# qwerty35/swarm_simulator

Hardware: AMD Instinct MI355X
Metric: agent-trajectories/sec (RBP plan: SFC+RSFC+QP) (higher is better)
Workload: dtype f64

## Files before the change

swarm_simulator_amd/csrc/kernels/knot_lds.inc:

```
#pragma once
#include "knot_panel_layout.h"

#define KL_LD 38
#define KL_LDU 50
#define KL_I 40
#ifndef KL_XCH
#define KL_XCH 6
#endif
typedef __attribute__((address_space(3))) double kl_lds;
typedef __attribute__((address_space(3))) int kl_ldsi;
typedef double kl_d2 __attribute__((ext_vector_type(2)));
typedef __attribute__((address_space(3))) kl_d2 kl_lds2;
typedef double kl_d4 __attribute__((ext_vector_type(4)));

__host__ __device__ constexpr int kl_area_doubles(int nk) {
    return ((nk + 1) * KL_LDU + (nk + 1) * KL_LD + KL_I + 1) & ~1;
}

template <int NK>
struct KlArea {
    static constexpr int NT = (NK + 15) / 16;
    static constexpr int C = 0, CSZ = (NK + 1) * KL_LDU;
    static constexpr int MX = CSZ, MXSZ = (NK + 1) * KL_LD;
    static constexpr int I = MX + MXSZ;
// ... 122 lines not shown
    }
}

#ifndef KL_FOLLOW_STRIDE
#define KL_FOLLOW_STRIDE 2
#endif
template <int NK>
__device__ __forceinline__ void kl_follow_LinvT(double (&m)[NK], const kl_lds* C, const kl_lds* I, kl_ldsi* P, int pbase) {
    double v[NK];
    kl_await_opaque(P, pbase + (KL_FOLLOW_STRIDE + 1 < NK ? KL_FOLLOW_STRIDE + 1 : NK));
    kl_load_tail<NK>(v, C, 1);
#pragma unroll
    for (int c = 0; c + 1 < NK; ++c) {
        if (c > 0 && c % KL_FOLLOW_STRIDE == 0) kl_await_opaque(P, pbase + (c + KL_FOLLOW_STRIDE + 1 < NK ? c + KL_FOLLOW_STRIDE + 1 : NK));
        const double s = m[c] * I[c];
        kl_axpy_roll<NK>(m, s, v, c + 1, C + (c + 1) * KL_LD, c + 2, c + 2 < NK);
    }
}

template <int NK>
__device__ __forceinline__ void kl_store_rows(const double (&m)[NK], kl_lds* MX, int r, bool act) {
    kl_lds* row = MX + (act ? r : NK) * KL_LD;
#pragma unroll
    for (int k = 0; k + 1 < NK; k += 2) *(kl_lds2*)(row + k) = kl_d2{m[k], m[k + 1]};
    if (NK & 1) row[NK - 1] = m[NK - 1];
    kl_sync();
}

template <int NK>
__device__ __forceinline__ void kl_coupling_rows(double (&x)[NK], kl_lds* MX, int r, bool act, double e0, double e1, double e2) {
    const int g3 = 3 * ((act ? r : 0) / 3);
    const kl_lds* m0 = MX + g3 * KL_LD;
    constexpr int NP = NK / 2;
    kl_d2 t[2][3][KL_XCH];
#pragma unroll
    for (int p = 0; p < KL_XCH && p < NP; ++p)
#pragma unroll
        for (int q = 0; q < 3; ++q) t[0][q][p] = *(const kl_lds2*)(m0 + q * KL_LD + 2 * p);
#pragma unroll
    for (int ch = 0; ch * KL_XCH < NP; ++ch) {
#pragma unroll
        for (int p = 0; p < KL_XCH; ++p)
            if ((ch + 1) * KL_XCH + p < NP)
#pragma unroll
                for (int q = 0; q < 3; ++q) t[(ch + 1) & 1][q][p] = *(const kl_lds2*)(m0 + q * KL_LD + 2 * ((ch + 1) * KL_XCH + p));
#pragma unroll
        for (int p = 0; p < KL_XCH; ++p) {
            const int k = 2 * (ch * KL_XCH + p);
            if (k + 1 < NK) {
                x[k] = e0 * t[ch & 1][0][p][0] + e1 * t[ch & 1][1][p][0] + e2 * t[ch & 1][2][p][0];
                x[k + 1] = e0 * t[ch & 1][0][p][1] + e1 * t[ch & 1][1][p][1] + e2 * t[ch & 1][2][p][1];
            }
        }
    }
    if (NK & 1) x[NK - 1] = e0 * m0[NK - 1] + e1 * m0[KL_LD + NK - 1] + e2 * m0[2 * KL_LD + NK - 1];
    kl_sync();
    kl_store_rows<NK>(x, MX, r, act);
}

template <int NK>
__device__ __forceinline__ void kl_syrk(const kl_lds* MX, const kl_lds* I, kl_lds* U, int lane, bool accumulate) {
    constexpr int NT = (NK + 15) / 16, KS = (NK + 3) / 4;
    const int li = lane & 15, lk = lane >> 4;
#pragma unroll
    for (int ti = 0; ti < NT; ++ti) {
        kl_d4 acc[NT];
#pragma unroll
        for (int t = 0; t < NT; ++t) acc[t] = kl_d4{0, 0, 0, 0};
        for (int ks = (3 * ((16 * ti) / 3)) / 4; ks < KS; ++ks) {
            const int kc = 4 * ks + lk;
            const double dk = kc < NK ? I[kc] : 0.0;
            const double opi = (kc < NK ? MX[(16 * ti + li < NK ? 16 * ti + li : NK) * KL_LD + kc] : 0.0) * dk;
#pragma unroll
            for (int tj = 0; tj <= ti; ++tj) {
                const double opj = kc < NK ? MX[(16 * tj + li < NK ? 16 * tj + li : NK) * KL_LD + kc] : 0.0;
                acc[tj] = __builtin_amdgcn_mfma_f64_16x16x4f64(opi, opj, acc[tj], 0, 0, 0);
            }
        }
#pragma unroll
        for (int tj = 0; tj <= ti; ++tj)
#pragma unroll
            for (int g = 0; g < 4; ++g) {
                const int row = 16 * ti + lk + 4 * g;
                kl_lds* u = U + (row < NK ? row : NK) * KL_LDU + 16 * tj + li;
                *u = accumulate ? *u + acc[tj][g] : acc[tj][g];
            }
    }
    kl_sync();
}

#ifndef KL_PANEL
#define KL_PANEL 1
#endif
#ifndef KL_PANEL_MIN_NK
#define KL_PANEL_MIN_NK 36
#endif
__host__ __device__ constexpr bool kl_panel_path(int nk) { return KL_PANEL && nk >= KL_PANEL_MIN_NK; }

template <int NK>
struct KlPanels {
    static constexpr int NT = kp_nt(NK), NP = kp_np(NK), TILES = kp_ntiles(NT);
    static_assert(kp_img_total(NK) <= KlArea<NK>::CSZ, "the panel images must fit the C / U region");
};

__device__ __forceinline__ double kl_recip(double d) {
    const double inv = __builtin_amdgcn_rcp(d);
    return __builtin_fma(__builtin_fma(-d, inv, 1.0), inv, inv);
}
__device__ __forceinline__ double kl_pick(bool c, double a, double b) {
    const long long m = -(long long)c;
    return __longlong_as_double((__double_as_longlong(a) & m) | (__double_as_longlong(b) & ~m));
}
__device__ __forceinline__ double kl_sel4(const double (&v)[4], int k) {
    return kl_pick((k & 2) != 0, kl_pick((k & 1) != 0, v[3], v[2]), kl_pick((k & 1) != 0, v[1], v[0]));
}

struct KlPivot {
    double d0, d10, d11, d20, d21, d22, d30, d31, d32, d33;
    double i0, i1, i2, i3;
    double w10, w20, w21, w30, w31, w32;
    double l10, l20, l21, l30, l31, l32;
    bool ok;
};
__device__ __forceinline__ void kl_pivot_load(KlPivot& f, const kl_lds* img, int p) {
    const kl_lds* b = img + kp_img_entry(KP_W * p, 0);
    f.d0 = b[0];
    const kl_d2 r1 = *(const kl_lds2*)(b + 4), r2 = *(const kl_lds2*)(b + 8), r3 = *(const kl_lds2*)(b + 12), r3b = *(const kl_lds2*)(b + 14);
    f.d22 = b[10];
    f.d10 = r1[0], f.d11 = r1[1], f.d20 = r2[0], f.d21 = r2[1], f.d30 = r3[0], f.d31 = r3[1], f.d32 = r3b[0], f.d33 = r3b[1];
}
__device__ __forceinline__ void kl_pivot_factor(KlPivot& f) {
    f.i0 = kl_recip(f.d0);
    f.w10 = f.d10, f.l10 = f.w10 * f.i0;
    f.w20 = f.d20, f.l20 = f.w20 * f.i0;
    f.w30 = f.d30, f.l30 = f.w30 * f.i0;
    const double d1 = __builtin_fma(-f.l10, f.w10, f.d11);
    f.i1 = kl_recip(d1);
    f.w21 = __builtin_fma(-f.l20, f.w10, f.d21), f.l21 = f.w21 * f.i1;
    f.w31 = __builtin_fma(-f.l30, f.w10, f.d31), f.l31 = f.w31 * f.i1;
    const double d2 = __builtin_fma(-f.l21, f.w21, __builtin_fma(-f.l20, f.w20, f.d22));
    f.i2 = kl_recip(d2);
    f.w32 = __builtin_fma(-f.l31, f.w21, __builtin_fma(-f.l30, f.w20, f.d32)), f.l32 = f.w32 * f.i2;
    const double d3 = __builtin_fma(-f.l32, f.w32, __builtin_fma(-f.l31, f.w31, __builtin_fma(-f.l30, f.w30, f.d33)));
    f.i3 = kl_recip(d3);
    f.ok = f.d0 > 0 && d1 > 0 && d2 > 0 && d3 > 0;
}
__device__ __forceinline__ void kl_panel_row(const KlPivot& f, const kl_d2 s01, const kl_d2 s23, double (&L)[4], double (&W)[4]) {
    W[0] = s01[0], L[0] = W[0] * f.i0;
    W[1] = __builtin_fma(-L[0], f.w10, s01[1]), L[1] = W[1] * f.i1;
    W[2] = __builtin_fma(-L[1], f.w21, __builtin_fma(-L[0], f.w20, s23[0])), L[2] = W[2] * f.i2;
    W[3] = __builtin_fma(-L[2], f.w32, __builtin_fma(-L[1], f.w31, __builtin_fma(-L[0], f.w30, s23[1]))), L[3] = W[3] * f.i3;
}

template <int NK, bool SUB, bool BOTH, class F>
__device__ __forceinline__ void kl_tiles_load(kl_d4 (&s)[KlPanels<NK>::TILES], int lane, F&& entry) {
    constexpr int NT = KlPanels<NK>::NT;
    const int li = lane & 15, lk = lane >> 4;
#pragma unroll
    for (int ti = 0; ti < NT; ++ti)
#pragma unroll
        for (int tj = ti; tj < NT; ++tj)
#pragma unroll
            for (int g = 0; g < 4; ++g) {
                const int i = KP_T * ti + lk + 4 * g, j = KP_T * tj + li;
                const int mx = BOTH ? j : i > j ? i : j, mn = BOTH ? i : i > j ? j : i;
                const bool full = KP_T * tj + KP_T <= NK;
                const bool pad = !full && (i >= NK || j >= NK);
                const double v = entry(full || mx < NK ? mx : NK - 1, full || mn < NK ? mn : NK - 1);
                const int tile = kp_upper(ti, tj, NT);
                if (SUB)
                    s[tile][g] -= pad ? 0.0 : v;
                else
                    s[tile][g] = pad ? (i == j ? 1.0 : 0.0) : v;
            }
}

template <int NK>
__device__ __forceinline__ void kl_panel_out(const kl_d4 (&s)[KlPanels<NK>::TILES], kl_lds* C, int p, int li, int lk) {
    constexpr int NT = KlPanels<NK>::NT;
    kl_lds* img = C + kp_img_off(NK, p);
#pragma unroll
    for (int tj = 0; tj < NT; ++tj)
        if (tj >= kp_panel_tile(p)) img[kp_img_entry(KP_T * tj + li, lk)] = s[kp_upper(kp_panel_tile(p), tj, NT)][kp_panel_reg(p)];
}

template <int NK>
__device__ __forceinline__ void kl_rows_load(kl_d2 (&raw)[KlPanels<NK>::NT][2], const kl_lds* img, int t_first, int li) {
#pragma unroll
    for (int t = 0; t < KlPanels<NK>::NT; ++t)
        if (t >= t_first) raw[t][0] = *(const kl_lds2*)(img + kp_img_entry(KP_T * t + li, 0)), raw[t][1] = *(const kl_lds2*)(img + kp_img_entry(KP_T * t + li, 2));
}

template <int NK>
__device__ __forceinline__ bool kl_ldl_panels(kl_d4 (&s)[KlPanels<NK>::TILES], kl_lds* C, kl_lds* I, int lane, kl_ldsi* P, int pbase) {
    constexpr int NT = KlPanels<NK>::NT, NP = KlPanels<NK>::NP;
    const int li = lane & 15, lk = lane >> 4;
    bool ok = true;
    KlPivot f;
    kl_d2 raw[NT][2];
    kl_panel_out<NK>(s, C, 0, li, lk);
    kl_sync();
    kl_pivot_load(f, C, 0);
    kl_rows_load<NK>(raw, C, 0, li);
#pragma unroll
    for (int p = 0; p < NP; ++p) {
        const int tc = kp_panel_tile(p), t0 = kp_first_live_tile(p);
        kl_lds* img = C + kp_img_off(NK, p);
        kl_pivot_factor(f);
        ok = ok && f.ok;
        if (KP_W * p + 0 < NK) I[KP_W * p + 0] = f.i0;
        if (KP_W * p + 1 < NK) I[KP_W * p + 1] = f.i1;
        if (KP_W * p + 2 < NK) I[KP_W * p + 2] = f.i2;
        if (KP_W * p + 3 < NK) I[KP_W * p + 3] = f.i3;
        const double inv[4] = {f.i0, f.i1, f.i2, f.i3};
        const double isel = kl_sel4(inv, lk);
        double a[NT], b[NT];
#pragma unroll
        for (int t = 0; t < NT; ++t)
            if (t >= tc) {
                double L[4], W[4];
                kl_panel_row(f, raw[t][0], raw[t][1], L, W);
                b[t] = kl_sel4(W, lk);
                const double l = b[t] * isel;
                a[t] = -l;
                img[kp_img_entry(KP_T * t + li, lk)] = l;
            }
        if (p + 1 < NP) {
#pragma unroll
            for (int tj = 0; tj < NT; ++tj)
                if (tj >= t0) s[kp_upper(t0, tj, NT)] = __builtin_amdgcn_mfma_f64_16x16x4f64(a[t0], b[tj], s[kp_upper(t0, tj, NT)], 0, 0, 0);
        }
        kl_sync();
        kl_publish(P, pbase + p + 1);
        if (p + 1 < NP) {
            kl_panel_out<NK>(s, C, p + 1, li, lk);
            kl_sync();
            kl_pivot_load(f, C + kp_img_off(NK, p + 1), p + 1);
            kl_rows_load<NK>(raw, C + kp_img_off(NK, p + 1), kp_panel_tile(p + 1), li);
            __builtin_amdgcn_sched_barrier(0);
#pragma unroll
            for (int ti = 0; ti < NT; ++ti)
#pragma unroll
                for (int tj = ti; tj < NT; ++tj)
                    if (ti > t0) s[kp_upper(ti, tj, NT)] = __builtin_amdgcn_mfma_f64_16x16x4f64(a[ti], b[tj], s[kp_upper(ti, tj, NT)], 0, 0, 0);
        }
    }
    kl_publish(P, pbase + NK + 1);
    return ok;
}

template <int NK, bool T_BOTH, class TF, class LF>
__device__ __forceinline__ bool kl_knot_panels(TF&& t_entry, LF&& t_loaded, bool minus_u, kl_lds* C, kl_lds* I, int lane, kl_ldsi* P, int pbase) {
    kl_d4 s[KlPanels<NK>::TILES];
    kl_tiles_load<NK, false, T_BOTH>(s, lane, t_entry);
    t_loaded();
    if (minus_u) kl_tiles_load<NK, true, true>(s, lane, [&](int mx, int mn) { return (double)C[mx * KL_LDU + mn]; });
    kl_sync();
    return kl_ldl_panels<NK>(s, C, I, lane, P, pbase);
}

template <int NK, bool WAIT>
__device__ __forceinline__ void kl_inverse_panels(kl_d4 (&n)[KlPanels<NK>::TILES], const kl_lds* C, int lane, kl_ldsi* P, int pbase) {
    constexpr int NT = KlPanels<NK>::NT, NP = KlPanels<NK>::NP;
    const int li = lane & 15, lk = lane >> 4;
#pragma unroll
    for (int ti = 0; ti < NT; ++ti)
#pragma unroll
        for (int tj = 0; tj <= ti; ++tj)
#pragma unroll
            for (int g = 0; g < 4; ++g) n[kp_lower(ti, tj)][g] = (ti == tj && lk + 4 * g == li) ? 1.0 : 0.0;
#pragma unroll
    for (int p = 0; p < NP; ++p) {
        const int tc = kp_panel_tile(p), q = kp_panel_reg(p);
        if (WAIT) kl_await_opaque(P, pbase + p + 1);
        const kl_lds* img = C + kp_img_off(NK, p);
        const kl_lds* bl = img + kp_img_entry(KP_W * p, 0);
        const double l10 = bl[4], l32 = bl[14];
        const kl_d2 r2 = *(const kl_lds2*)(bl + 8), r3 = *(const kl_lds2*)(bl + 12);
        kl_d2 raw[NT][2];
        kl_rows_load<NK>(raw, img, tc, li);
        const double l20 = r2[0], l21 = r2[1], l30 = r3[0], l31 = r3[1];
        const double k10 = -l10, k21 = -l21, k32 = -l32;
        const double k20 = __builtin_fma(-l21, k10, -l20), k31 = __builtin_fma(-l32, k21, -l31);
        const double k30 = __builtin_fma(-l32, k20, __builtin_fma(-l31, k10, -l30));
        double a[NT], b[NT];
#pragma unroll
        for (int t = 0; t < NT; ++t)
            if (t >= tc) {
                const double L[4] = {raw[t][0][0], raw[t][0][1], raw[t][1][0], raw[t][1][1]};
                double G[4];
                G[3] = -L[3];
                G[2] = -__builtin_fma(L[3], k32, L[2]);
                G[1] = -__builtin_fma(L[3], k31, __builtin_fma(L[2], k21, L[1]));
                G[0] = -__builtin_fma(L[3], k30, __builtin_fma(L[2], k20, __builtin_fma(L[1], k10, L[0])));
                if (t == tc) {
                    const int ar = KP_T * t + li - KP_W * p;
                    G[0] = kl_pick(ar >= 4, G[0], kl_pick(ar == 1, k10, kl_pick(ar == 2, k20, kl_pick(ar == 3, k30, 0.0))));
                    G[1] = kl_pick(ar >= 4, G[1], kl_pick(ar == 2, k21, kl_pick(ar == 3, k31, 0.0)));
                    G[2] = kl_pick(ar >= 4, G[2], kl_pick(ar == 3, k32, 0.0));
                    G[3] = kl_pick(ar >= 4, G[3], 0.0);
                }
                a[t] = kl_sel4(G, lk);
            }
#pragma unroll
        for (int tj = 0; tj < NT; ++tj)
            if (tj <= tc) b[tj] = n[kp_lower(tc, tj)][q];
#pragma unroll
        for (int ti = 0; ti < NT; ++ti)
#pragma unroll
            for (int tj = 0; tj <= ti; ++tj)
                if (ti >= tc && tj <= tc) n[kp_lower(ti, tj)] = __builtin_amdgcn_mfma_f64_16x16x4f64(a[ti], b[tj], n[kp_lower(ti, tj)], 0, 0, 0);
    }
}

template <int NK>
__device__ __forceinline__ void kl_tiles_to_rows(const kl_d4 (&n)[KlPanels<NK>::TILES], double (&m)[NK], kl_lds* MX, int lane, int r, bool act) {
    constexpr int NT = KlPanels<NK>::NT;
    const int li = lane & 15, lk = lane >> 4;
#pragma unroll
    for (int ti = 0; ti < NT; ++ti)
#pragma unroll
        for (int tj = 0; tj < NT; ++tj)
#pragma unroll
            for (int g = 0; g < 4; ++g) {
                if (KP_T * ti + 4 * g >= NK) continue;
                const int col = KP_T * ti + lk + 4 * g, row = KP_T * tj + li;
                const bool in = (KP_T * tj + KP_T <= NK || row < NK) && (KP_T * ti + 4 * g + 4 <= NK || col < NK);
                MX[in ? row * KL_LD + col : NK * KL_LD + li] = tj <= ti ? n[kp_lower(ti, tj)][g] : 0.0;
            }
    kl_sync();
    const kl_lds* row = MX + (act ? r : NK) * KL_LD;
#pragma unroll
    for (int k = 0; k + 1 < NK; k += 2) {
        const kl_d2 t = *(const kl_lds2*)(row + k);
        m[k] = t[0], m[k + 1] = t[1];
    }
    if (NK & 1) m[NK - 1] = row[NK - 1];
    kl_sync();
}

template <int NK, bool FOLLOW>
__device__ __forceinline__ double kl_inverse_rows(double (&m)[NK], const kl_lds* C, const kl_lds* I, kl_lds* MX, int r, bool act, kl_ldsi* P, int pbase) {
    if constexpr (kl_panel_path(NK)) {
        kl_d4 n[KlPanels<NK>::TILES];
        kl_inverse_panels<NK, FOLLOW>(n, C, r, P, pbase);
        kl_tiles_to_rows<NK>(n, m, MX, r, r, act);
        if (FOLLOW) kl_await_opaque(P, pbase + NK + 1);
        return I[act ? r : 0];
    } else {
#pragma unroll
        for (int k = 0; k < NK; ++k) m[k] = (k == r) ? 1.0 : 0.0;
        if (FOLLOW)
            kl_follow_LinvT<NK>(m, C, I, P, pbase);
        else
            kl_row_times_LinvT<NK>(m, C, I);
        if (FOLLOW) kl_await_opaque(P, pbase + NK + 1);
        const double dinv = I[act ? r : 0];
        kl_store_rows<NK>(m, MX, r, act);
        return dinv;
    }
}
```

swarm_simulator_amd/csrc/kernels/knot_panel_layout.h:

```cpp
#pragma once
#ifndef KP_FN
#define KP_FN __host__ __device__ inline
#endif

#define KP_W 4
#define KP_T 16

KP_FN constexpr int kp_nt(int nk) { return (nk + KP_T - 1) / KP_T; }
KP_FN constexpr int kp_np(int nk) { return (nk + KP_W - 1) / KP_W; }
KP_FN constexpr int kp_rows(int nk) { return KP_T * kp_nt(nk); }

KP_FN constexpr int kp_a_row(int lane) { return lane & 15; }
KP_FN constexpr int kp_a_k(int lane) { return lane >> 4; }
KP_FN constexpr int kp_b_col(int lane) { return lane & 15; }
KP_FN constexpr int kp_b_k(int lane) { return lane >> 4; }
KP_FN constexpr int kp_cd_col(int lane) { return lane & 15; }
KP_FN constexpr int kp_cd_row(int lane, int reg) { return (lane >> 4) + 4 * reg; }

KP_FN constexpr int kp_ntiles(int nt) { return nt * (nt + 1) / 2; }
KP_FN constexpr int kp_upper(int ti, int tj, int nt) { return ti * nt - ti * (ti - 1) / 2 + (tj - ti); }
KP_FN constexpr int kp_lower(int ti, int tj) { return ti * (ti + 1) / 2 + tj; }

KP_FN constexpr int kp_panel_tile(int p) { return p / (KP_T / KP_W); }
KP_FN constexpr int kp_panel_reg(int p) { return p % (KP_T / KP_W); }
KP_FN constexpr int kp_first_live_tile(int p) { return kp_panel_tile(p + 1); }

KP_FN constexpr int kp_img_doubles(int nk) { return kp_rows(nk) * KP_W; }
KP_FN constexpr int kp_img_off(int nk, int p) { return p * kp_img_doubles(nk); }
KP_FN constexpr int kp_img_entry(int row, int k) { return row * KP_W + k; }
KP_FN constexpr int kp_img_total(int nk) { return kp_np(nk) * kp_img_doubles(nk); }
```

swarm_simulator_amd/csrc/kernels/qp.hip:

```cpp
#include <algorithm>
#include <type_traits>
#include <vector>

#include "rbp_dev.h"

#pragma clang fp contract(fast)

#include "knot_lds.inc"

#ifndef QP_THREADS
#define QP_THREADS 512
#endif
#define QP_MAX_ITERS 80
#ifndef QP_POLISH_FIRST
#define QP_POLISH_FIRST 1
#endif
#ifndef QP_WARM_TAU
#define QP_WARM_TAU 1e-3
#endif
#ifndef QP_MU0
#define QP_MU0 3e-1
#endif
#ifndef QP_UNI_POLISH
#define QP_UNI_POLISH 1
// ... 1068 lines not shown
    for (int u = 0; u * 64 < per; ++u) {
        const int t = lane + 64 * u;
        if (t < per) {
            int Ai = (int)(((2 * n3 + 1) - sqrtf((float)((2 * n3 + 1) * (2 * n3 + 1) - 8 * t))) * 0.5f);
            if (Ai * n3 - Ai * (Ai - 1) / 2 > t) Ai--;
            if ((Ai + 1) * n3 - (Ai + 1) * Ai / 2 <= t) Ai++;
            const int Bi = Ai + t - (Ai * n3 - Ai * (Ai - 1) / 2);
            const int a = Ai / 3, k = Ai % 3, b = Bi / 3, l = Bi % 3;
            double Sv[6];
            if (a == b) {
                const int kk = k < l ? k : l, ll = k < l ? l : k, sym = kk == 0 ? ll : (kk == 1 ? 2 + ll : 5);
#pragma unroll
                for (int pp = 0; pp < 6; ++pp) Sv[pp] = Sin[(a * 6 + sym) * 6 + pp];
            } else {
                const int pw = a * nb - a * (a + 1) / 2 + (b - a - 1);
#pragma unroll
                for (int pp = 0; pp < 6; ++pp)
                    Sv[pp] = -Pw[pw * 6 + pp] * (double)Nr[(pw * 2 + (pp >= 3)) * 3 + k] * (double)Nr[(pw * 2 + (pp >= 3)) * 3 + l];
            }
#pragma unroll
            for (int e = 0; e < 3; ++e)
#pragma unroll
                for (int f = 0; f < 3; ++f) {
                    double acc = Sv[0] * L[e] * L[f] + Sv[1] * L[3 + e] * L[3 + f] + Sv[2] * L[6 + e] * L[6 + f];
                    if (e == f) acc += Sv[3 + e];
                    if (Ai == Bi) acc += Dk[3 * e + f];
                    Timg[(3 * Ai + e) * KL_LD + 3 * Bi + f] = acc;
                    Timg[(3 * Bi + f) * KL_LD + 3 * Ai + e] = acc;
                }
        }
    }
    kl_sync();
}
__device__ void assemble_blocks_lds(const AsmArgs& A, int nj, double* lds) {
    const int wave = threadIdx.x >> 6, NW = QP_THREADS / 64;
    int j = wave - NW;
    assemble_knots_lds<true>(A, lds + (size_t)wave * ASML_DOUBLES(9 * A.nb, A.nb), [&] { j += NW; return j < nj ? j : -1; }, [](int) {});
}

__device__ inline AsmArgs asm_args(const RowCtx& c) {
    return AsmArgs{c.w.cpacc, c.w.pwgt, c.w.Lk, c.w.Dk, c.normals, c.w.Td, c.d.N, c.d.M, c.d.nb, c.d.first, c.d.oq, c.d.ldb};
}

__device__ void assemble_blocks(const RowCtx& c, double* lds) {
    const QpDims& d = c.d;
    const QpWs& w = c.w;
    const int nk = d.nk, oq = d.oq, nb = d.nb, lb = d.ldb;
    const AsmArgs A = asm_args(c);
    const bool in_lds = nb * oq * 6 <= c.lds_avail;
    if (in_lds) {
        for (int it = threadIdx.x; it < nb * oq * 6; it += QP_THREADS) lds[it] = w.cpacc[(size_t)(it % 6) * (nb * oq) + it / 6];
        __syncthreads();
    }
    const int per_knot = nb * nb * 9;
    for (int it = threadIdx.x; it < d.nj * per_knot; it += QP_THREADS) assemble_item(A, in_lds ? lds : nullptr, it / per_knot + 1, it % per_knot);
    if (d.nj > 1 && nk > 36 && 3 * lb * (lb + 2) > c.lds_avail) {
        const size_t noff = (size_t)(d.nj - 1) * lb * lb;
        for (size_t it = threadIdx.x; it < noff; it += QP_THREADS) {
            const int j = (int)(it / ((size_t)lb * lb)) + 1;
            const int rr = (int)(it % ((size_t)lb * lb)) / lb, cc = (int)(it % ((size_t)lb * lb)) % lb;
            double v = 0;
            if (rr / 3 == cc / 3 && rr < nk && cc < nk) v = w.Ek[9 * j + 3 * (cc % 3) + (rr % 3)];
            w.To[it] = v;
        }
    }
}

__device__ __forceinline__ double rl(double v, int lane) {
    int lo = __builtin_amdgcn_readlane(__double2loint(v), lane);
    int hi = __builtin_amdgcn_readlane(__double2hiint(v), lane);
    return __hiloint2double(hi, lo);
}

__device__ __forceinline__ int twist_mid(int nj) { return nj / 2; }

#define ASM_WAVE0 4
#define ASM_HELPERS (QP_THREADS / 64 > ASM_WAVE0 ? QP_THREADS / 64 - ASM_WAVE0 : 0)
#ifndef QP_FOLLOW_ASM
#define QP_FOLLOW_ASM (ASM_HELPERS == 0)
#endif
#define ASMF_READY(cnt, h) ((kl_ldsi*)((cnt) + 76 + (h)))
__device__ __forceinline__ void wait_blocks(int* cnt, int i) {
    while (__hip_atomic_load(cnt + i, __ATOMIC_RELAXED, __HIP_MEMORY_SCOPE_WORKGROUP) < ASM_HELPERS) __builtin_amdgcn_s_sleep(2);
    __builtin_amdgcn_fence(__ATOMIC_ACQUIRE, "workgroup");
}

typedef double d4 __attribute__((ext_vector_type(4)));

template <int NK>
__device__ __forceinline__ bool chol_rows(double (&a)[NK], double& dinv) {
    bool ok = true;
    const int r = threadIdx.x & 63;
    dinv = 1.0;
#pragma unroll
    for (int c = 0; c < NK; ++c) {
        const double dcc = rl(a[c], c);
        if (!(dcc > 0)) ok = false;
        const double inv = fast_rsqrt(dcc);
        dinv = (r == c) ? inv : dinv;
        a[c] *= inv;
#pragma unroll
        for (int k = c + 1; k < NK; ++k) a[k] -= a[c] * rl(a[c], k);
    }
    return ok;
}

#define KF_STRIDE(NK) ((NK) * (NK) + KL_I)

__device__ __forceinline__ void coupling_coef(const QpWs& w, int j, int dir, int rr, double& e0, double& e1, double& e2) {
    const __attribute__((address_space(1))) double* E = QGC(w.Ek) + 9 * (dir > 0 ? j + 1 : j);
    e0 = dir > 0 ? E[rr % 3] : E[3 * (rr % 3)], e1 = dir > 0 ? E[3 + rr % 3] : E[3 * (rr % 3) + 1],
    e2 = dir > 0 ? E[6 + rr % 3] : E[3 * (rr % 3) + 2];
}

template <int NK>
__device__ __forceinline__ bool knot_ldl(const QpWs& w, int j, bool minus_u, kl_lds* base, int r, bool act, int rr, kl_ldsi* P, int pbase,
                                         const kl_lds* Timg = nullptr, kl_ldsi* consumed = nullptr, int consumed_value = 0) {
    using A = KlArea<NK>;
    kl_lds *C = base + A::C, *I = base + A::I, *U = base + A::C;
    if constexpr (kl_panel_path(NK)) {
        if (Timg)
            return kl_knot_panels<NK, true>([&](int mx, int mn) { return (double)Timg[mn * KL_LD + mx]; },
                                      [&] {
                                          kl_sync();
                                          if (consumed) kl_publish(consumed, consumed_value);
                                      },
                                      minus_u, C, I, r, P, pbase);
        const double* Tg = w.Td + (size_t)j * NK * NK;
        return kl_knot_panels<NK, false>([&](int mx, int mn) { return Tg[mn * NK + mx]; }, [] {}, minus_u, C, I, r, P, pbase);
    }
    double a[NK];
    if (Timg) {
#pragma unroll
        for (int k = 0; k < NK; ++k) a[k] = Timg[k * KL_LD + rr];
        kl_sync();
        if (consumed) kl_publish(consumed, consumed_value);
    } else {
        const double* Tg = w.Td + (size_t)j * NK * NK;
#pragma unroll
#ifdef QP_T_HALF_ROWS
        for (int k = 0; k < NK; ++k) a[k] = Tg[k * NK + (rr > k ? rr : k)];
#else
        for (int k = 0; k < NK; ++k) a[k] = Tg[k * NK + rr];
#endif
    }
    if (minus_u) {
#pragma unroll
        for (int k = 0; k < NK; ++k) a[k] -= U[rr * KL_LDU + k];
        kl_sync();
    }
    return kl_ldl<NK>(a, C, I, r, act, P, pbase);
}

template <int NK, bool FOLLOW>
__device__ __forceinline__ void knot_inverse(const QpWs& w, int j, kl_lds* base, int r, bool act, kl_ldsi* P, int pbase, int& seen, kl_ldsi* Mdone,
                                             int done_value) {
    using A = KlArea<NK>;
    kl_lds *C = base + A::C, *MX = base + A::MX, *I = base + A::I;
    double m[NK];
    const double dinv = kl_inverse_rows<NK, FOLLOW>(m, C, I, MX, r, act, P, pbase);
    if (FOLLOW) kl_publish(Mdone, done_value);
    __attribute__((address_space(1))) double* Mg = QG(w.Lf + (size_t)j * KF_STRIDE(NK));
    if (FOLLOW && QP_FOLLOW_ASM) asm volatile("s_waitcnt vmcnt(0)" ::: "memory");
    if (act) {
        __attribute__((address_space(1))) double* row = Mg + (size_t)r * NK;
        if ((NK & 1) == 0) {
#pragma unroll
            for (int k = 0; k < NK; k += 2)
                if (k + 1 >= r) *(__attribute__((address_space(1))) kl_d2*)(row + k) = kl_d2{m[k], m[k + 1]};
        } else {
#pragma unroll
            for (int k = 0; k < NK; ++k)
                if (k >= r) row[k] = m[k];
        }
        Mg[NK * NK + r] = dinv;
    }
}

#if defined(QP_PROFILE) && !defined(QP_LHSTATS) && !defined(QP_SOLVE_TIMERS)
#define CHAIN_T0 long long ct_ = wall_clock64()
#define CHAIN_T(slot)                                                          \
    do {                                                                       \
        const long long t_ = wall_clock64();                                   \
        if (w.prof && dir > 0 && r == 0) w.prof[slot] += (double)(t_ - ct_);   \
        ct_ = t_;                                                              \
    } while (0)
#else
#define CHAIN_T0
#define CHAIN_T(slot)
#endif
#define CHAIN_SYNC(cnt, h) ((kl_ldsi*)((cnt) + 64 + 2 * (h)))
#define ASM_CONSUMED(cnt, h) ((kl_ldsi*)((cnt) + 72 + (h)))

template <int NK>
__device__ __forceinline__ bool wave_factor_chain(const QpDims& d, const QpWs& w, int j0, int count, int dir, double* ldsW, int* cnt, int h) {
    using A = KlArea<NK>;
    kl_lds* base = (kl_lds*)ldsW;
    kl_lds *MX = base + A::MX, *I = base + A::I, *U = base + A::C;
    kl_ldsi *P = CHAIN_SYNC(cnt, h), *Mdone = P + 1;
    const int r = threadIdx.x & 63;
    const bool act = r < NK;
    const int rr = act ? r : 0;
    bool ok = true;
    int seen = 0, seen_img = 0;
    for (int i = 0, j = j0; i < count; ++i, j += dir) {
        CHAIN_T0;
        if (i > 0) kl_syrk<NK>(MX, I, U, r, false);
        CHAIN_T(25);
        if (QP_FOLLOW_ASM)
            kl_await(ASMF_READY(cnt, h), i + 1, seen_img);
        else
            wait_blocks(cnt, i);
        CHAIN_T(26);
        double e0, e1, e2, x[NK];
        coupling_coef(w, j, dir, rr, e0, e1, e2);
        const kl_lds* Timg = ASM_HELPERS > 0 ? (const kl_lds*)(ldsW - (size_t)h * A::SIZE + 2 * A::SIZE + 128 + (size_t)(h + 2 * (i & 1)) * ASML_DOUBLES(NK, (NK / 9)))
                             : QP_FOLLOW_ASM ? (const kl_lds*)(ldsW - (size_t)h * A::SIZE + 2 * A::SIZE + 128 + (size_t)h * ASML_DOUBLES(NK, (NK / 9)))
                                             : nullptr;
        if (!knot_ldl<NK>(w, j, i > 0, base, r, act, rr, P, i * (NK + 1), Timg, ASM_CONSUMED(cnt, h), i + 1)) ok = false;
        kl_await(Mdone, i + 1, seen);
        kl_coupling_rows<NK>(x, MX, r, act, e0, e1, e2);
        CHAIN_T(27);
    }
    return ok;
}

template <int NK>
__device__ __forceinline__ bool wave_factor_mid(const QpDims& d, const QpWs& w, double* ldsL, double* ldsR, int* cnt, int cnt_idx) {
    using A = KlArea<NK>;
    kl_lds *bl = (kl_lds*)ldsL, *br = (kl_lds*)ldsR;
    const int r = threadIdx.x & 63, mid = twist_mid(d.nj);
    const bool act = r < NK;
    const int rr = act ? r : 0;
    int nsy = 0;
    if (mid > 0) kl_syrk<NK>(bl + A::MX, bl + A::I, bl + A::C, r, false), nsy++;
    if (mid + 1 < d.nj) kl_syrk<NK>(br + A::MX, br + A::I, bl + A::C, r, nsy > 0), nsy++;
    if (QP_FOLLOW_ASM) {
        int seen_img = 0;
        kl_await(ASMF_READY(cnt, 0), mid + 1, seen_img);
    } else {
        wait_blocks(cnt, cnt_idx);
    }
    kl_ldsi* scratch = CHAIN_SYNC(cnt, 2);
    const kl_lds* Timg = ASM_HELPERS > 0 ? (const kl_lds*)(ldsL + 2 * A::SIZE + 128 + (size_t)(2 * (cnt_idx & 1)) * ASML_DOUBLES(NK, (NK / 9)))
                         : QP_FOLLOW_ASM ? (const kl_lds*)(ldsL + 2 * A::SIZE + 128) : nullptr;
    const bool ok = knot_ldl<NK>(w, mid, nsy > 0, bl, r, act, rr, scratch, 0, Timg);
    if (!QP_MID_FOLLOW) {
        int seen = 0;
        knot_inverse<NK, false>(w, mid, bl, r, act, scratch, 0, seen, scratch, 0);
    }
    return ok;
}

template <int NK, int ROLE>
__device__ __forceinline__ bool twisted_factor(const QpDims& d, const QpWs& w, int* flag, double* lds, const AsmArgs* asmb) {
    const int wave = (ROLE == 0 || ROLE == 2) ? (threadIdx.x >> 6) & 1 : 4, mid = twist_mid(d.nj);
    const int nl = mid, nr = d.nj - 1 - mid, SF = nl > nr ? nl : nr;
    constexpr int AREA = KlArea<NK>::SIZE;
    int* cnt = (int*)(lds + 2 * AREA);
    static_assert((QP_MAX_M - 1) / 2 + 1 <= 64, "cnt[0..SF] must end below CHAIN_SYNC (cnt + 64): sessions with M > QP_MAX_M are refused");
    if (threadIdx.x == 0) *flag = 0;
    __syncthreads();
    bool ok = true;
    for (int i = threadIdx.x; i < 2 * AREA + 64; i += QP_THREADS) lds[i] = 0.0;
    __syncthreads();
    if (ROLE == 0) {
        __builtin_amdgcn_s_setprio(QP_CHAIN_PRIO);
        if (wave == 0 && mid > 0) ok = wave_factor_chain<NK>(d, w, 0, mid, +1, lds, cnt, 0);
        if (wave == 1 && nr > 0) ok = wave_factor_chain<NK>(d, w, d.nj - 1, nr, -1, lds + AREA, cnt, 1);
        if (wave == 1) __builtin_amdgcn_s_setprio(0);
    }
    if (ROLE == 1) {
        const AsmArgs A = *asmb;
        const int hw = (threadIdx.x >> 6) - ASM_WAVE0, side = hw & 1, par = hw >> 1;
        double* scratch = lds + 2 * AREA + 128 + (size_t)hw * ASML_DOUBLES(NK, (NK / 9));
        int i = par - 2;
        kl_ldsi* consumed = ASM_CONSUMED(cnt, side);
        int seen_c = 0;
        assemble_knots_lds<false>(
            A, scratch,
            [&] {
                for (i += 2; i <= SF; i += 2) {
                    const bool work = i < SF ? (side ? i < nr : i < nl) : side == 0;
                    if (work) {
                        if (i >= 2) kl_await(consumed, i - 1, seen_c);
                        return i < SF ? (side ? d.nj - 1 - i : i) : mid;
                    }
                    if ((threadIdx.x & 63) == 0)
                        __hip_atomic_fetch_add(cnt + i, i < SF ? ASM_HELPERS / 2 : 0, __ATOMIC_RELAXED, __HIP_MEMORY_SCOPE_WORKGROUP);
                }
                return -1;
            },
            [&](int) {
                __builtin_amdgcn_fence(__ATOMIC_RELEASE, "workgroup");
                if ((threadIdx.x & 63) == 0)
                    __hip_atomic_fetch_add(cnt + i, i < SF ? ASM_HELPERS / 2 : ASM_HELPERS, __ATOMIC_RELAXED, __HIP_MEMORY_SCOPE_WORKGROUP);
            });
    }
    if (ROLE == 2) {
        const int count = wave == 0 ? nl : nr, j0 = wave == 0 ? 0 : d.nj - 1, dir = wave == 0 ? +1 : -1;
        kl_lds* base = (kl_lds*)(lds + wave * AREA);
        kl_ldsi *P = CHAIN_SYNC(cnt, wave), *Mdone = P + 1;
        const int r = threadIdx.x & 63;
        int seen = 0;
        if (QP_FOLLOW_ASM) {
            const AsmArgs A = *asmb;
            double* scratch = lds + 2 * AREA + 128 + (size_t)wave * ASML_DOUBLES(NK, (NK / 9));
            kl_ldsi *ready = ASMF_READY(cnt, wave), *consumed = ASM_CONSUMED(cnt, wave);
            const int total = count + (wave == 0 ? 1 : 0);
            int seen_c = 0;
            auto blk = [&](int n) { return n < count ? j0 + n * dir : mid; };
            auto make = [&](int n) {
                if (n > 0) kl_await(consumed, n, seen_c);
                fasm_tiles(A, scratch, blk(n));
                __builtin_amdgcn_fence(__ATOMIC_RELEASE, "workgroup");
                kl_publish(ready, n + 1);
                if (n + 1 < total) fasm_fetch(A, scratch, blk(n + 1));
            };
            if (total > 0) {
                fasm_fetch(A, scratch, blk(0));
                make(0);
            }
            for (int i = 0; i < count; ++i) {
                knot_inverse<NK, true>(w, j0 + i * dir, base, r, r < NK, P, i * (NK + 1), seen, Mdone, i + 1);
                if (i + 1 < total) make(i + 1);
            }
        } else {
            for (int i = 0; i < count; ++i) knot_inverse<NK, true>(w, j0 + i * dir, base, r, r < NK, P, i * (NK + 1), seen, Mdone, i + 1);
        }
    }
    if (!ok && (threadIdx.x & 63) == 0) atomicExch(flag, 1);
    __threadfence_block();
    __syncthreads();
    if (*flag) return false;
    if (ROLE == 0 && wave == 0) {
        if (!wave_factor_mid<NK>(d, w, lds, lds + AREA, cnt, SF) && threadIdx.x == 0) *flag = 1;
        __builtin_amdgcn_s_setprio(0);
    }
    if (QP_MID_FOLLOW && ROLE == 2 && wave == 0) {
        const int r = threadIdx.x & 63;
        int seen = 0;
        kl_ldsi* P = CHAIN_SYNC(cnt, 2);
        knot_inverse<NK, true>(w, mid, (kl_lds*)lds, r, r < NK, P, 0, seen, P + 1, 1);
    }
    __threadfence_block();
    __syncthreads();
    return *flag == 0;
}

#define KS_VPAD 16
#define KS_VLEN (KS_VPAD + KL_I + KS_VPAD)
template <int NK>
struct KsPieces {
    static constexpr int CH = (NK * 15 + 35) / 36;
    static constexpr int N0 = NK, N1 = NK - CH > 0 ? NK - CH : 0, N2 = NK - 2 * CH > 0 ? NK - 2 * CH : 0;
    static_assert(NK - 3 * CH <= 0 && N0 + N1 + N2 <= 64, "three chunks, one wavefront");
    static_assert(3 * CH - NK <= KS_VPAD && 3 * CH - 1 - (NK - 1) <= KS_VPAD, "vector padding");
    __device__ static __forceinline__ void of_lane(int lane, int& idx, int& t) {
        t = lane < N0 ? 0 : (lane < N0 + N1 ? 1 : 2);
        idx = lane < N0 ? lane : (lane < N0 + N1 ? lane - N0 : (lane < N0 + N1 + N2 ? lane - N0 - N1 : 0));
    }
};
template <int NK>
__device__ __forceinline__ double kl_matvec_cols(const kl_lds* Mst, const kl_lds* b, kl_lds* psum, int lane) {
    using P = KsPieces<NK>;
    int idx, t;
    P::of_lane(lane, idx, t);
    const int k0 = P::CH * t, c = k0 + idx;
    const kl_lds* mp = Mst + k0 * KL_LD + c;
    const kl_lds* bp = b + k0;
    double mv[P::CH], bv[P::CH];
#pragma unroll
    for (int j = 0; j < P::CH; ++j) mv[j] = mp[j * KL_LD], bv[j] = bp[j];
    double s0 = 0, s1 = 0, s2 = 0;
#pragma unroll
    for (int j = 0; j < P::CH; ++j) {
        if (j % 3 == 0) s0 += mv[j] * bv[j];
        if (j % 3 == 1) s1 += mv[j] * bv[j];
        if (j % 3 == 2) s2 += mv[j] * bv[j];
    }
    psum[lane] = (s0 + s1) + s2;
    kl_sync();
    const int cc = lane < NK ? lane : 0;
    double r = psum[cc];
    if (P::N1 > 0) r += cc >= P::CH ? psum[P::N0 + cc - P::CH] : 0.0;
    if (P::N2 > 0) r += cc >= 2 * P::CH ? psum[P::N0 + P::N1 + cc - 2 * P::CH] : 0.0;
    return r;
}
template <int NK>
__device__ __forceinline__ double kl_matvec_rows(const kl_lds* Mst, const kl_lds* b, kl_lds* psum, int lane) {
    using P = KsPieces<NK>;
    int idx, t;
    P::of_lane(lane, idx, t);
    const int k0 = NK - P::CH * (t + 1);
    const kl_lds* mp = Mst + idx * KL_LD + k0;
    const kl_lds* bp = b + k0;
    double mv[P::CH], bv[P::CH];
#pragma unroll
    for (int j = 0; j < P::CH; ++j) mv[j] = mp[j], bv[j] = bp[j];
// ... 1953 lines not shown
```

Measured before the change: 177,500.

## Fuse Schur-complement update into MFMA panel tiles before LDL factorization

On the panel path, the coupling update (previously a separate syrk that wrote the update into LDS, plus separate coupling-row computation) now accumulates directly into register-resident MFMA tiles. Coupling coefficients are folded into the A/B operands, and the next block's T matrix is then added in place. The inverse's Mdone publish moves earlier, and one LDS barrier after the row load is dropped, so the next chain step can start sooner. Profiling timers now go through LDS atomics. The change adds register pressure from holding tiles across the wait, and it alters the ordering of synchronisation between waves.

```diff
diff --git a/swarm_simulator_amd/csrc/kernels/knot_lds.inc b/swarm_simulator_amd/csrc/kernels/knot_lds.inc
--- a/swarm_simulator_amd/csrc/kernels/knot_lds.inc
+++ b/swarm_simulator_amd/csrc/kernels/knot_lds.inc
@@ -298,7 +298,7 @@
     W[3] = __builtin_fma(-L[2], f.w32, __builtin_fma(-L[1], f.w31, __builtin_fma(-L[0], f.w30, s23[1]))), L[3] = W[3] * f.i3;
 }
 
-template <int NK, bool SUB, bool BOTH, class F>
+template <int NK, int OP, bool BOTH, class F>
 __device__ __forceinline__ void kl_tiles_load(kl_d4 (&s)[KlPanels<NK>::TILES], int lane, F&& entry) {
     constexpr int NT = KlPanels<NK>::NT;
     const int li = lane & 15, lk = lane >> 4;
@@ -314,8 +314,10 @@
                 const bool pad = !full && (i >= NK || j >= NK);
                 const double v = entry(full || mx < NK ? mx : NK - 1, full || mn < NK ? mn : NK - 1);
                 const int tile = kp_upper(ti, tj, NT);
-                if (SUB)
+                if (OP == 1)
                     s[tile][g] -= pad ? 0.0 : v;
+                else if (OP == 2)
+                    s[tile][g] = pad ? (i == j ? 1.0 : 0.0) : s[tile][g] + v;
                 else
                     s[tile][g] = pad ? (i == j ? 1.0 : 0.0) : v;
             }
@@ -398,10 +400,86 @@
 template <int NK, bool T_BOTH, class TF, class LF>
 __device__ __forceinline__ bool kl_knot_panels(TF&& t_entry, LF&& t_loaded, bool minus_u, kl_lds* C, kl_lds* I, int lane, kl_ldsi* P, int pbase) {
     kl_d4 s[KlPanels<NK>::TILES];
-    kl_tiles_load<NK, false, T_BOTH>(s, lane, t_entry);
+    kl_tiles_load<NK, 0, T_BOTH>(s, lane, t_entry);
     t_loaded();
-    if (minus_u) kl_tiles_load<NK, true, true>(s, lane, [&](int mx, int mn) { return (double)C[mx * KL_LDU + mn]; });
-    kl_sync();
+    if (minus_u) kl_tiles_load<NK, 1, true>(s, lane, [&](int mx, int mn) { return (double)C[mx * KL_LDU + mn]; });
+    kl_sync();
+    return kl_ldl_panels<NK>(s, C, I, lane, P, pbase);
+}
+
+#ifndef KL_FUSED_UPDATE
+#define KL_FUSED_UPDATE 1
+#endif
+__host__ __device__ constexpr bool kl_fused_path(int nk) { return KL_FUSED_UPDATE && kl_panel_path(nk); }
+
+template <int NK, class F>
+__device__ __forceinline__ void kl_fused_coef(double (&cf)[KlPanels<NK>::NT][3], int lane, F&& coef) {
+    const int li = lane & 15;
+#pragma unroll
+    for (int t = 0; t < KlPanels<NK>::NT; ++t) {
+        const int row = KP_T * t + li;
+        const bool in = KP_T * t + KP_T <= NK || row < NK;
+#pragma unroll
+        for (int q = 0; q < 3; ++q) {
+            const double c = coef(in ? row : 0, q);
+            cf[t][q] = in ? c : 0.0;
+        }
+    }
+}
+
+template <int NK>
+__device__ __forceinline__ void kl_tiles_zero(kl_d4 (&s)[KlPanels<NK>::TILES]) {
+#pragma unroll
+    for (int t = 0; t < KlPanels<NK>::TILES; ++t) s[t] = kl_d4{0, 0, 0, 0};
+}
+
+template <int NK, bool SKIP = true>
+__device__ __forceinline__ void kl_fused_update(kl_d4 (&s)[KlPanels<NK>::TILES], const kl_lds* MX, const kl_lds* I, int lane, const double (&cf)[KlPanels<NK>::NT][3]) {
+    constexpr int NT = KlPanels<NK>::NT, KS = kp_ksteps(NK);
+    const int li = lane & 15, lk = lane >> 4;
+    const kl_lds* grp[NT];
+#pragma unroll
+    for (int t = 0; t < NT; ++t) {
+        const int row = KP_T * t + li;
+        grp[t] = MX + kp_x_group(KP_T * t + KP_T <= NK || row < NK ? row : 0) * KL_LD + lk;
+    }
+    double raw[2][NT][3], dk[2];
+    auto request = [&](int ks) {
+        const bool live = KP_W * ks + KP_W <= NK || KP_W * ks + lk < NK;
+        dk[ks & 1] = I[live ? KP_W * ks + lk : 0];
+#pragma unroll
+        for (int t = 0; t < NT; ++t)
+            if (!SKIP || ks >= kp_x_first_kstep(t))
+#pragma unroll
+                for (int q = 0; q < 3; ++q) raw[ks & 1][t][q] = grp[t][q * KL_LD + KP_W * ks];
+    };
+    request(0);
+#pragma unroll
+    for (int ks = 0; ks < KS; ++ks) {
+        if (ks + 1 < KS) request(ks + 1);
+        const bool live = KP_W * ks + KP_W <= NK || KP_W * ks + lk < NK;
+        double a[NT], b[NT];
+#pragma unroll
+        for (int t = 0; t < NT; ++t)
+            if (!SKIP || ks >= kp_x_first_kstep(t)) {
+                const double (&m)[3] = raw[ks & 1][t];
+                const double x = cf[t][0] * m[0] + cf[t][1] * m[1] + cf[t][2] * m[2];
+                a[t] = live ? -x : 0.0;
+                b[t] = live ? x * dk[ks & 1] : 0.0;
+            }
+#pragma unroll
+        for (int tj = 0; tj < NT; ++tj)
+            if (!SKIP || ks >= kp_x_first_kstep(tj))
+#pragma unroll
+                for (int ti = 0; ti <= tj; ++ti)
+                    s[kp_upper(ti, tj, NT)] = __builtin_amdgcn_mfma_f64_16x16x4f64(a[ti], b[tj], s[kp_upper(ti, tj, NT)], 0, 0, 0);
+    }
+}
+
+template <int NK, bool T_BOTH, class TF, class LF>
+__device__ __forceinline__ bool kl_knot_panels_add(kl_d4 (&s)[KlPanels<NK>::TILES], TF&& t_entry, LF&& t_loaded, kl_lds* C, kl_lds* I, int lane, kl_ldsi* P, int pbase) {
+    kl_tiles_load<NK, 2, T_BOTH>(s, lane, t_entry);
+    t_loaded();
     return kl_ldl_panels<NK>(s, C, I, lane, P, pbase);
 }
 
@@ -460,7 +538,7 @@
 }
 
 template <int NK>
-__device__ __forceinline__ void kl_tiles_to_rows(const kl_d4 (&n)[KlPanels<NK>::TILES], double (&m)[NK], kl_lds* MX, int lane, int r, bool act) {
+__device__ __forceinline__ void kl_tiles_scatter(const kl_d4 (&n)[KlPanels<NK>::TILES], kl_lds* MX, int lane) {
     constexpr int NT = KlPanels<NK>::NT;
     const int li = lane & 15, lk = lane >> 4;
 #pragma unroll
@@ -475,6 +553,9 @@
                 MX[in ? row * KL_LD + col : NK * KL_LD + li] = tj <= ti ? n[kp_lower(ti, tj)][g] : 0.0;
             }
     kl_sync();
+}
+template <int NK>
+__device__ __forceinline__ void kl_row_load(double (&m)[NK], const kl_lds* MX, int r, bool act) {
     const kl_lds* row = MX + (act ? r : NK) * KL_LD;
 #pragma unroll
     for (int k = 0; k + 1 < NK; k += 2) {
@@ -482,17 +563,29 @@
         m[k] = t[0], m[k + 1] = t[1];
     }
     if (NK & 1) m[NK - 1] = row[NK - 1];
-    kl_sync();
 }
 
 template <int NK, bool FOLLOW>
-__device__ __forceinline__ double kl_inverse_rows(double (&m)[NK], const kl_lds* C, const kl_lds* I, kl_lds* MX, int r, bool act, kl_ldsi* P, int pbase) {
+__device__ __forceinline__ double kl_inverse_rows(double (&m)[NK], const kl_lds* C, const kl_lds* I, kl_lds* MX, int r, bool act, kl_ldsi* P, int pbase,
+                                                  kl_ldsi* Mdone = nullptr, int done_value = 0) {
     if constexpr (kl_panel_path(NK)) {
         kl_d4 n[KlPanels<NK>::TILES];
         kl_inverse_panels<NK, FOLLOW>(n, C, r, P, pbase);
-        kl_tiles_to_rows<NK>(n, m, MX, r, r, act);
+        kl_tiles_scatter<NK>(n, MX, r);
+        if (kl_fused_path(NK)) {
+            if (FOLLOW) kl_await_opaque(P, pbase + NK + 1);
+            const double dinv = I[act ? r : 0];
+            __builtin_amdgcn_fence(__ATOMIC_RELEASE, "wavefront");
+            if (FOLLOW) kl_publish(Mdone, done_value);
+            kl_row_load<NK>(m, MX, r, act);
+            return dinv;
+        }
+        kl_row_load<NK>(m, MX, r, act);
+        kl_sync();
         if (FOLLOW) kl_await_opaque(P, pbase + NK + 1);
-        return I[act ? r : 0];
+        const double dinv = I[act ? r : 0];
+        if (FOLLOW) kl_publish(Mdone, done_value);
+        return dinv;
     } else {
 #pragma unroll
         for (int k = 0; k < NK; ++k) m[k] = (k == r) ? 1.0 : 0.0;
@@ -503,6 +596,7 @@
         if (FOLLOW) kl_await_opaque(P, pbase + NK + 1);
         const double dinv = I[act ? r : 0];
         kl_store_rows<NK>(m, MX, r, act);
+        if (FOLLOW) kl_publish(Mdone, done_value);
         return dinv;
     }
 }
diff --git a/swarm_simulator_amd/csrc/kernels/knot_panel_layout.h b/swarm_simulator_amd/csrc/kernels/knot_panel_layout.h
--- a/swarm_simulator_amd/csrc/kernels/knot_panel_layout.h
+++ b/swarm_simulator_amd/csrc/kernels/knot_panel_layout.h
@@ -25,6 +25,10 @@
 KP_FN constexpr int kp_panel_reg(int p) { return p % (KP_T / KP_W); }
 KP_FN constexpr int kp_first_live_tile(int p) { return kp_panel_tile(p + 1); }
 
+KP_FN constexpr int kp_x_group(int row) { return 3 * (row / 3); }
+KP_FN constexpr int kp_x_first_kstep(int t) { return kp_x_group(KP_T * t) / KP_W; }
+KP_FN constexpr int kp_ksteps(int nk) { return (nk + KP_W - 1) / KP_W; }
+
 KP_FN constexpr int kp_img_doubles(int nk) { return kp_rows(nk) * KP_W; }
 KP_FN constexpr int kp_img_off(int nk, int p) { return p * kp_img_doubles(nk); }
 KP_FN constexpr int kp_img_entry(int row, int k) { return row * KP_W + k; }
diff --git a/swarm_simulator_amd/csrc/kernels/qp.hip b/swarm_simulator_amd/csrc/kernels/qp.hip
--- a/swarm_simulator_amd/csrc/kernels/qp.hip
+++ b/swarm_simulator_amd/csrc/kernels/qp.hip
@@ -1244,14 +1244,34 @@
     return kl_ldl<NK>(a, C, I, r, act, P, pbase);
 }
 
+template <int NK>
+__device__ __forceinline__ bool knot_ldl_add(const QpWs& w, int j, kl_d4 (&s)[KlPanels<NK>::TILES], kl_lds* base, int r, kl_ldsi* P, int pbase,
+                                             const kl_lds* Timg = nullptr, kl_ldsi* consumed = nullptr, int consumed_value = 0) {
+    using A = KlArea<NK>;
+    kl_lds *C = base + A::C, *I = base + A::I;
+    if (Timg)
+        return kl_knot_panels_add<NK, true>(s, [&](int mx, int mn) { return (double)Timg[mn * KL_LD + mx]; },
+                                            [&] {
+                                                kl_sync();
+                                                if (consumed) kl_publish(consumed, consumed_value);
+                                            },
+                                            C, I, r, P, pbase);
+    const double* Tg = w.Td + (size_t)j * NK * NK;
+    return kl_knot_panels_add<NK, false>(s, [&](int mx, int mn) { return Tg[mn * NK + mx]; }, [] {}, C, I, r, P, pbase);
+}
+template <int NK>
+__device__ __forceinline__ void fused_coupling_coef(const QpWs& w, int j, int dir, int lane, double (&cf)[KlPanels<NK>::NT][3]) {
+    const __attribute__((address_space(1))) double* E = QGC(w.Ek) + 9 * (dir > 0 ? j + 1 : j);
+    kl_fused_coef<NK>(cf, lane, [&](int row, int q) { return dir > 0 ? E[3 * q + row % 3] : E[3 * (row % 3) + q]; });
+}
+
 template <int NK, bool FOLLOW>
 __device__ __forceinline__ void knot_inverse(const QpWs& w, int j, kl_lds* base, int r, bool act, kl_ldsi* P, int pbase, int& seen, kl_ldsi* Mdone,
                                              int done_value) {
     using A = KlArea<NK>;
     kl_lds *C = base + A::C, *MX = base + A::MX, *I = base + A::I;
     double m[NK];
-    const double dinv = kl_inverse_rows<NK, FOLLOW>(m, C, I, MX, r, act, P, pbase);
-    if (FOLLOW) kl_publish(Mdone, done_value);
+    const double dinv = kl_inverse_rows<NK, FOLLOW>(m, C, I, MX, r, act, P, pbase, Mdone, done_value);
     __attribute__((address_space(1))) double* Mg = QG(w.Lf + (size_t)j * KF_STRIDE(NK));
     if (FOLLOW && QP_FOLLOW_ASM) asm volatile("s_waitcnt vmcnt(0)" ::: "memory");
     if (act) {
@@ -1270,16 +1290,24 @@
 }
 
 #if defined(QP_PROFILE) && !defined(QP_LHSTATS) && !defined(QP_SOLVE_TIMERS)
+#define CHAIN_TW(cnt, slot) ((__attribute__((address_space(3))) unsigned long long*)((cnt) + 96) + ((slot) - 25))
 #define CHAIN_T0 long long ct_ = wall_clock64()
-#define CHAIN_T(slot)                                                          \
-    do {                                                                       \
-        const long long t_ = wall_clock64();                                   \
-        if (w.prof && dir > 0 && r == 0) w.prof[slot] += (double)(t_ - ct_);   \
-        ct_ = t_;                                                              \
+#define CHAIN_T(slot)                                                                                                                              \
+    do {                                                                                                                                           \
+        const long long t_ = wall_clock64();                                                                                                       \
+        __hip_atomic_fetch_add(CHAIN_TW(cnt, slot), (dir > 0 && r == 0) ? (unsigned long long)(t_ - ct_) : 0ull, __ATOMIC_RELAXED, __HIP_MEMORY_SCOPE_WORKGROUP); \
+        ct_ = t_;                                                                                                                                  \
+    } while (0)
+#define CHAIN_FLUSH()                                                                                   \
+    do {                                                                                                \
+        kl_sync();                                                                                      \
+        if (w.prof && dir > 0 && r == 0)                                                                \
+            for (int k_ = 25; k_ < 28; ++k_) w.prof[k_] += (double)(long long)*CHAIN_TW(cnt, k_);       \
     } while (0)
 #else
 #define CHAIN_T0
 #define CHAIN_T(slot)
+#define CHAIN_FLUSH()
 #endif
 #define CHAIN_SYNC(cnt, h) ((kl_ldsi*)((cnt) + 64 + 2 * (h)))
 #define ASM_CONSUMED(cnt, h) ((kl_ldsi*)((cnt) + 72 + (h)))
@@ -1295,6 +1323,33 @@
     const int rr = act ? r : 0;
     bool ok = true;
     int seen = 0, seen_img = 0;
+    if constexpr (kl_fused_path(NK)) {
+        double cf[KlPanels<NK>::NT][3];
+        for (int i = 0, j = j0; i < count; ++i, j += dir) {
+            CHAIN_T0;
+            kl_d4 s[KlPanels<NK>::TILES];
+            kl_tiles_zero<NK>(s);
+            if (i > 0) {
+                kl_await(Mdone, i, seen);
+                CHAIN_T(27);
+                kl_fused_update<NK>(s, MX, I, r, cf);
+            }
+            CHAIN_T(25);
+            if (QP_FOLLOW_ASM)
+                kl_await(ASMF_READY(cnt, h), i + 1, seen_img);
+            else
+                wait_blocks(cnt, i);
+            CHAIN_T(26);
+            fused_coupling_coef<NK>(w, j, dir, r, cf);
+            const kl_lds* Timg = ASM_HELPERS > 0 ? (const kl_lds*)(ldsW - (size_t)h * A::SIZE + 2 * A::SIZE + 128 + (size_t)(h + 2 * (i & 1)) * ASML_DOUBLES(NK, (NK / 9)))
+                                 : QP_FOLLOW_ASM ? (const kl_lds*)(ldsW - (size_t)h * A::SIZE + 2 * A::SIZE + 128 + (size_t)h * ASML_DOUBLES(NK, (NK / 9)))
+                                                 : nullptr;
+            if (!knot_ldl_add<NK>(w, j, s, base, r, P, i * (NK + 1), Timg, ASM_CONSUMED(cnt, h), i + 1)) ok = false;
+            CHAIN_T(27);
+        }
+        CHAIN_FLUSH();
+        return ok;
+    }
     for (int i = 0, j = j0; i < count; ++i, j += dir) {
         CHAIN_T0;
         if (i > 0) kl_syrk<NK>(MX, I, U, r, false);
@@ -1314,6 +1369,7 @@
         kl_coupling_rows<NK>(x, MX, r, act, e0, e1, e2);
         CHAIN_T(27);
     }
+    CHAIN_FLUSH();
     return ok;
 }
 
@@ -1325,8 +1381,28 @@
     const bool act = r < NK;
     const int rr = act ? r : 0;
     int nsy = 0;
-    if (mid > 0) kl_syrk<NK>(bl + A::MX, bl + A::I, bl + A::C, r, false), nsy++;
-    if (mid + 1 < d.nj) kl_syrk<NK>(br + A::MX, br + A::I, bl + A::C, r, nsy > 0), nsy++;
+    [[maybe_unused]] kl_d4 s[kl_fused_path(NK) ? KlPanels<NK>::TILES : 1];
+    if constexpr (kl_fused_path(NK)) {
+        double cl[KlPanels<NK>::NT][3], cr[KlPanels<NK>::NT][3];
+        if (mid > 0) fused_coupling_coef<NK>(w, mid - 1, +1, r, cl);
+        if (mid + 1 < d.nj) fused_coupling_coef<NK>(w, mid + 1, -1, r, cr);
+        kl_tiles_zero<NK>(s);
+        if (mid > 0) kl_fused_update<NK>(s, bl + A::MX, bl + A::I, r, cl);
+        if (mid + 1 < d.nj) {
+            if (mid > 0) {
+                kl_d4 s2[KlPanels<NK>::TILES];
+                kl_tiles_zero<NK>(s2);
+                kl_fused_update<NK>(s2, br + A::MX, br + A::I, r, cr);
+#pragma unroll
+                for (int t = 0; t < KlPanels<NK>::TILES; ++t) s[t] += s2[t];
+            } else {
+                kl_fused_update<NK>(s, br + A::MX, br + A::I, r, cr);
+            }
+        }
+    } else {
+        if (mid > 0) kl_syrk<NK>(bl + A::MX, bl + A::I, bl + A::C, r, false), nsy++;
+        if (mid + 1 < d.nj) kl_syrk<NK>(br + A::MX, br + A::I, bl + A::C, r, nsy > 0), nsy++;
+    }
     if (QP_FOLLOW_ASM) {
         int seen_img = 0;
         kl_await(ASMF_READY(cnt, 0), mid + 1, seen_img);
@@ -1336,7 +1412,11 @@
     kl_ldsi* scratch = CHAIN_SYNC(cnt, 2);
     const kl_lds* Timg = ASM_HELPERS > 0 ? (const kl_lds*)(ldsL + 2 * A::SIZE + 128 + (size_t)(2 * (cnt_idx & 1)) * ASML_DOUBLES(NK, (NK / 9)))
                          : QP_FOLLOW_ASM ? (const kl_lds*)(ldsL + 2 * A::SIZE + 128) : nullptr;
-    const bool ok = knot_ldl<NK>(w, mid, nsy > 0, bl, r, act, rr, scratch, 0, Timg);
+    bool ok;
+    if constexpr (kl_fused_path(NK))
+        ok = knot_ldl_add<NK>(w, mid, s, bl, r, scratch, 0, Timg);
+    else
+        ok = knot_ldl<NK>(w, mid, nsy > 0, bl, r, act, rr, scratch, 0, Timg);
     if (!QP_MID_FOLLOW) {
         int seen = 0;
         knot_inverse<NK, false>(w, mid, bl, r, act, scratch, 0, seen, scratch, 0);
```

New measurement: 179,800, median of 6. 1.01x the previous value.
